# cosmicBboy/movenet

Measured on AMD Instinct MI355X. Metric: autoregressive audio samples/sec (16 kHz, 30-layer WaveNet, whole job), higher is better.
Workload: dtype f32

## Files before the change

movenet_amd/csrc/generate_fold.hip:

```cpp
#include <cstdlib>

#include "common.h"
#include "gen_common.h"
#include "pipe_common.h"

namespace mvn {

namespace fold {
constexpr int C = 64, Q = 256, NT = 512, LPS = 3;
constexpr int KQ = 4, KPER = 16, NF4 = 4;
constexpr int MAT_F = 2 * C * C;
enum { M_A0 = 0, M_A0P, M_A1, M_A2, M_B2P,
       M_B1, M_B1P, M_B2, M_RR, M_RS,
       M_WP0, M_WP1, M_WP2, M_SS,
       N_MAT };
constexpr int N_LDS_MAT = 4;
constexpr int V_CB1 = 0, V_CB2 = 2 * C, V_BSP = 4 * C, V_BR0 = 5 * C, V_BS0 = 6 * C, V_BR1 = 7 * C,
              V_BS1 = 8 * C, V_BR2 = 9 * C, VEC_F = 10 * C;
constexpr int STAGE_F = N_MAT * MAT_F + VEC_F;
constexpr int CTX_LAYER_F = MAT_F + 2 * C;
constexpr int EMB_F = 2 * Q * C;
constexpr int W1_F = Q * C, W2_F = Q * Q, WSL_F = C * C;
constexpr int HEAD_F = W1_F + Q + W2_F + Q + WSL_F + C;
constexpr int GRAN = 3 * C;
constexpr int LDS_FLOATS = N_LDS_MAT * MAT_F + 1536 + 16;
constexpr int GMAX = 8;
constexpr int PFS_F = 8;
constexpr int LDS_FLOATS_MULTI = LDS_FLOATS + GMAX * C * PFS_F;
}

struct FoldMat {
  v2f w[16];
};
__device__ __forceinline__ void fold_load(FoldMat &m, const float *sec, int t) {
#pragma unroll
  for (int i = 0; i < 8; ++i) {
    const f4 v = ((const f4 *)sec)[i * 256 + t];
    m.w[2 * i] = v2f{v.x, v.y};
    m.w[2 * i + 1] = v2f{v.z, v.w};
  }
}
__device__ __forceinline__ v2f pk_fma_hi(v2f w, v2f xpair, v2f acc) {
  asm("v_pk_fma_f32 %0, %1, %2, %0 op_sel:[0,1,0]" : "+v"(acc) : "v"(w), "v"(xpair));
  return acc;
}
__device__ __forceinline__ v2f pk_mul_hi(v2f w, v2f xpair) {
  v2f r;
  asm("v_pk_mul_f32 %0, %1, %2 op_sel:[0,1]" : "=v"(r) : "v"(w), "v"(xpair));
  return r;
}
template <bool INIT>
__device__ __forceinline__ void pair_acc(v2f (&acc)[4], const v2f (&w)[16], const f4 (&x)[4]) {
#pragma unroll
  for (int i = 0; i < 4; ++i) {
    if (INIT && i == 0) {
      acc[0] = w[0] * v2f{x[0].x, x[0].x};
      acc[1] = w[1] * v2f{x[0].y, x[0].y};
      acc[2] = w[2] * v2f{x[0].z, x[0].z};
      acc[3] = pk_mul_hi(w[3], v2f{x[0].z, x[0].w});
    } else {
      acc[0] = __builtin_elementwise_fma(w[4 * i], v2f{x[i].x, x[i].x}, acc[0]);
      acc[1] = __builtin_elementwise_fma(w[4 * i + 1], v2f{x[i].y, x[i].y}, acc[1]);
      acc[2] = __builtin_elementwise_fma(w[4 * i + 2], v2f{x[i].z, x[i].z}, acc[2]);
      acc[3] = pk_fma_hi(w[4 * i + 3], v2f{x[i].z, x[i].w}, acc[3]);
    }
  }
}
__device__ __forceinline__ v2f pair_sum(const v2f (&acc)[4]) { return (acc[0] + acc[2]) + (acc[1] + acc[3]); }
template <int H>
__device__ __forceinline__ float split_dot(const v2f (&w)[16], const f4 (&x)[4]) {
  v2f a0 = w[8 * H] * v2f{x[0].x, x[0].y}, a1 = w[8 * H + 1] * v2f{x[0].z, x[0].w};
  v2f a2 = w[8 * H + 2] * v2f{x[1].x, x[1].y}, a3 = w[8 * H + 3] * v2f{x[1].z, x[1].w};
  a0 = __builtin_elementwise_fma(w[8 * H + 4], v2f{x[2].x, x[2].y}, a0);
  a1 = __builtin_elementwise_fma(w[8 * H + 5], v2f{x[2].z, x[2].w}, a1);
  a2 = __builtin_elementwise_fma(w[8 * H + 6], v2f{x[3].x, x[3].y}, a2);
  a3 = __builtin_elementwise_fma(w[8 * H + 7], v2f{x[3].z, x[3].w}, a3);
  const v2f t = (a0 + a2) + (a1 + a3);
  return t.x + t.y;
}

typedef __attribute__((address_space(3))) float lds_f;
typedef float vf4 __attribute__((ext_vector_type(4)));
typedef __attribute__((address_space(3))) vf4 lds_f4;
__device__ __forceinline__ f4 lds_load4(unsigned addr) {
  const vf4 v = *(const lds_f4 *)(uintptr_t)addr;
  f4 r;
  r.x = v.x; r.y = v.y; r.z = v.z; r.w = v.w;
  return r;
}
__device__ __forceinline__ unsigned lds_addr(const float *p) { return (unsigned)(uintptr_t)(lds_f *)p; }
#define LDSF(addr, off) (*(lds_f *)(uintptr_t)((addr) + 4u * (unsigned)(off)))
template <int N4>
__device__ __forceinline__ void ldsv(f4 (&x)[N4], unsigned addr, int off) {
#pragma unroll
  for (int i = 0; i < N4; ++i) x[i] = lds_load4(addr + 4u * (unsigned)off + 16u * i);
}

__device__ __forceinline__ v2f pair_dot_lds(unsigned waddr, unsigned xaddr) {
  v2f acc[4];
#pragma unroll
  for (int i = 0; i < 4; ++i) {
    const f4 wa = lds_load4(waddr + 4096u * (2 * i)), wb = lds_load4(waddr + 4096u * (2 * i + 1));
    const f4 x = lds_load4(xaddr + 16u * i);
    if (i == 0) {
      acc[0] = v2f{wa.x, wa.y} * v2f{x.x, x.x};
      acc[1] = v2f{wa.z, wa.w} * v2f{x.y, x.y};
      acc[2] = v2f{wb.x, wb.y} * v2f{x.z, x.z};
      acc[3] = pk_mul_hi(v2f{wb.z, wb.w}, v2f{x.z, x.w});
    } else {
      acc[0] = __builtin_elementwise_fma(v2f{wa.x, wa.y}, v2f{x.x, x.x}, acc[0]);
      acc[1] = __builtin_elementwise_fma(v2f{wa.z, wa.w}, v2f{x.y, x.y}, acc[1]);
      acc[2] = __builtin_elementwise_fma(v2f{wb.x, wb.y}, v2f{x.z, x.z}, acc[2]);
      acc[3] = pk_fma_hi(v2f{wb.z, wb.w}, v2f{x.z, x.w}, acc[3]);
    }
  }
  return pair_sum(acc);
}
template <int H>
__device__ __forceinline__ float split_dot_lds(unsigned waddr, unsigned xaddr) {
  f4 w[4], x[4];
#pragma unroll
  for (int i = 0; i < 4; ++i) {
    w[i] = lds_load4(waddr + 4096u * (4 * H + i));
    x[i] = lds_load4(xaddr + 16u * i);
  }
  v2f a0 = v2f{w[0].x, w[0].y} * v2f{x[0].x, x[0].y}, a1 = v2f{w[0].z, w[0].w} * v2f{x[0].z, x[0].w};
  v2f a2 = v2f{w[1].x, w[1].y} * v2f{x[1].x, x[1].y}, a3 = v2f{w[1].z, w[1].w} * v2f{x[1].z, x[1].w};
  a0 = __builtin_elementwise_fma(v2f{w[2].x, w[2].y}, v2f{x[2].x, x[2].y}, a0);
  a1 = __builtin_elementwise_fma(v2f{w[2].z, w[2].w}, v2f{x[2].z, x[2].w}, a1);
  a2 = __builtin_elementwise_fma(v2f{w[3].x, w[3].y}, v2f{x[3].x, x[3].y}, a2);
  a3 = __builtin_elementwise_fma(v2f{w[3].z, w[3].w}, v2f{x[3].z, x[3].w}, a3);
  const v2f t = (a0 + a2) + (a1 + a3);
  return t.x + t.y;
}

template <bool MULTI>
__global__ __launch_bounds__(512, 2) void gen_fold_kernel(GenArgs a, u64 *hand, unsigned *err, int NS, int nb, int nseq) {
  using namespace fold;
  extern __shared__ __attribute__((aligned(16))) float smem[];
  const int tid = threadIdx.x, lane = tid & 63, wave = tid >> 6;
  const int xcd = blockIdx.x & 7, slot = blockIdx.x >> 3;
  const int in_xcd = (PIPE_XCD_CUS / NS) * NS;
  int b, s;
  if (slot < in_xcd) {
    b = xcd + 8 * (slot / NS);
    s = slot % NS;
  } else {
    const int idx = xcd * (PIPE_XCD_CUS - in_xcd) + (slot - in_xcd);
    b = 8 * (PIPE_XCD_CUS / NS) + idx / NS;
    s = idx % NS;
  }
  if (b >= nb) return;
  if (__hip_atomic_load(err, __ATOMIC_RELAXED, __HIP_MEMORY_SCOPE_AGENT) != 0) return;
  const int L = a.L;
  const int s_next = s + 1 == NS ? 0 : s + 1;
  const int G = MULTI ? (nseq - b + nb - 1) / nb : 1;
  int bq = b;
  u64 *inbox = hand + ((size_t)b * NS + s) * GRAN;
  u64 *outbox = hand + ((size_t)b * NS + s_next) * GRAN;
  int *iflag = (int *)(smem + LDS_FLOATS - 16);
  float *pfs = smem + LDS_FLOATS;
  const bool fast_edge = pipe_edge_is_fast(err + 16, b, s, s_next, NS, iflag);

  if (s < NS - 1) {
    const int l0 = s * LPS, nl = min(LPS, L - l0);
    const bool chain = tid < 256;
    const int t = tid & 255, c = t >> 2, kq = t & 3;
    const bool lead = kq == 0;
    float *lmat = smem;
    constexpr int O_XP = 0;
    constexpr int O_ZL = C;
    constexpr int O_Z0 = 2 * C, O_Z1 = 3 * C;
    constexpr int O_X0 = 4 * C;
    constexpr int O_B1 = 5 * C, O_B2 = 7 * C;
    constexpr int O_PAST = 9 * C;
    constexpr int O_CTX = 12 * C;
    constexpr int O_VEC = 13 * C;
    float *vec = smem + N_LDS_MAT * MAT_F;
    unsigned vc = lds_addr(vec) + 4u * c;
    unsigned vq = lds_addr(vec) + 4u * KPER * kq;
    asm volatile("" : "+v"(vc), "+v"(vq));
    u64 *ob = outbox + c;
    const u64 *ibs = inbox + 2 * C + c;
    float *ring = a.state + (size_t)b * a.state_per_seq;
    auto bind = [&](int g) {
      bq = b + g * nb;
      inbox = hand + ((size_t)bq * NS + s) * GRAN;
      outbox = hand + ((size_t)bq * NS + s_next) * GRAN;
      ob = outbox + c;
      ibs = inbox + 2 * C + c;
      ring = a.state + (size_t)bq * a.state_per_seq;
    };
    const float *sec = a.w + EMB_F + (size_t)s * STAGE_F;
    const float *vecs = sec + N_MAT * MAT_F;

    FoldMat m0, m1, m2, m3, m4;
    {
      const int first = chain ? M_A0 : M_B1;
      fold_load(m0, sec + (size_t)(first + 0) * MAT_F, t);
      fold_load(m1, sec + (size_t)(first + 1) * MAT_F, t);
      fold_load(m2, sec + (size_t)(first + 2) * MAT_F, t);
      fold_load(m3, sec + (size_t)(first + 3) * MAT_F, t);
      fold_load(m4, sec + (size_t)(first + 4) * MAT_F, t);
      const f4 *src = (const f4 *)(sec + (size_t)M_WP0 * MAT_F);
      for (int i = tid; i < N_LDS_MAT * MAT_F / 4; i += NT) ((f4 *)lmat)[i] = src[i];
    }
    float pf[LPS], pg[LPS];
    float (&xs)[LPS] = pf;
    int doff[LPS], dmask[LPS];
    for (int i = tid; i < VEC_F; i += NT) vec[O_VEC + i] = vecs[i];
#pragma unroll
    for (int j = 0; j < LPS; ++j) {
      pf[j] = 0.f; pg[j] = 0.f;
      const int l = l0 + j;
      dmask[j] = j < nl ? (1 << (l % a.layer_size)) - 1 : 0;
      doff[j] = j < nl ? ring_offset(l, a.layer_size, C) : 0;
    }

    float popv[LPS] = {0.f, 0.f, 0.f};
    auto prefetch_pops = [&](int tn) {
      if (MULTI && !chain && lead) {
        int cq = c;
        asm volatile("" : "+v"(cq));
#pragma unroll
        for (int j = 0; j < LPS; ++j)
          if (j < nl) popv[j] = ring_load(ring + doff[j] + cq + (tn & dmask[j]) * C);
      }
    };
    auto precompute = [&](int tn, bool push, bool popped) {
      int tq = t;
      asm volatile("" : "+v"(tq));
      const int cq = tq >> 2, kk = tq & 3;
      if (!chain && lead) {
#pragma unroll
        for (int j = 0; j < LPS; ++j)
          if (j < nl) {
            float *base = ring + doff[j] + cq;
            if (push) base[((tn - 1) & dmask[j]) * C] = xs[j];
            const float pv = (push && dmask[j] == 0) ? xs[j]
                             : (MULTI && popped) ? popv[j] : ring_load(base + (tn & dmask[j]) * C);
            vec[O_PAST + j * C + cq] = pv;
          }
      }
      if (a.ctx_tm && chain && tq < C) vec[O_CTX + tq] = a.ctx_tm[(size_t)bq * a.ctx_stride_b + (size_t)tn * C + tq];
      __syncthreads();
      if (chain) {
        const unsigned wm = lds_addr(lmat) + 16u * tq, xq = lds_addr(vec) + 4u * (O_PAST + KPER * kk);
        const v2f p0 = pair_dot_lds(wm, xq);
        const v2f p1 = pair_dot_lds(wm + 4u * MAT_F, xq + 4u * C);
        const v2f p2 = pair_dot_lds(wm + 8u * MAT_F, xq + 8u * C);
        pf[0] = chan_sum<KQ>(p0.x);
        pg[0] = chan_sum<KQ>(p0.y);
        pf[1] = chan_sum<KQ>(p1.x) + vec[O_VEC + V_CB1 + cq];
        pg[1] = chan_sum<KQ>(p1.y) + vec[O_VEC + V_CB1 + C + cq];
        pf[2] = chan_sum<KQ>(p2.x) + vec[O_VEC + V_CB2 + cq];
        pg[2] = chan_sum<KQ>(p2.y) + vec[O_VEC + V_CB2 + C + cq];
        if (a.ctx_tm) {
#pragma unroll
          for (int j = 0; j < LPS; ++j)
            if (j < nl) {
              const float *wc = a.wctx + (size_t)(l0 + j) * CTX_LAYER_F;
              pf[j] += chan_sum<KQ>(dot_stream<NF4>((const f4 *)wc, 256, tq, vec + O_CTX + KPER * kk)) + wc[MAT_F + cq];
              pg[j] += chan_sum<KQ>(dot_stream<NF4>((const f4 *)wc + NF4 * 256, 256, tq, vec + O_CTX + KPER * kk)) +
                       wc[MAT_F + C + cq];
            }
        }
      }
    };
    auto save_pf = [&](int g) {
      if (MULTI && chain && lead) {
        float *q = pfs + ((size_t)g * C + c) * PFS_F;
        *(f4 *)q = f4{pf[0], pg[0], pf[1], pg[1]};
        *(v2f *)(q + 4) = v2f{pf[2], pg[2]};
      }
    };
    auto load_pf = [&](int g) {
      if (MULTI && chain) {
        const float *q = pfs + ((size_t)g * C + c) * PFS_F;
        const f4 v = *(const f4 *)q;
        const v2f w = *(const v2f *)(q + 4);
        pf[0] = v.x; pg[0] = v.y; pf[1] = v.z; pg[1] = v.w; pf[2] = w.x; pg[2] = w.y;
      }
    };
    __syncthreads();
    if (MULTI) {
      for (int g = 0; g < G; ++g) {
        bind(g);
        precompute(a.t_begin, false, false);
        save_pf(g);
        __syncthreads();
      }
    } else {
      precompute(a.t_begin, false, false);
    }

    bool alive = true;
    for (int ts = a.t_begin; ts < a.t_end && alive; ++ts)
    for (int g = 0; g < G; ++g) {
      if (MULTI) {
        bind(g);
        if (ts + 1 < a.t_end) prefetch_pops(ts + 1);
      }
      const unsigned epoch = (unsigned)(ts - a.t_begin + 1);
      if (wave == 0) {
        float v[2];
        const bool ok = wait_inbox<2>(inbox, epoch, err, v);
        if (ok) {
          float *dst = vec + 2 * lane;
          dst[0] = v[0];
          dst[1] = v[1];
        }
        if (lane == 0) iflag[0] = ok ? 1 : 0;
      }
      lds_barrier();
      MVN_STAMP(b, s, ts - a.t_begin, 0);
      load_pf(g);
      float xv = 0.f;
      MVN_FINE(b, s, ts - a.t_begin, 0, 0);
      if (chain) {
        f4 xa[NF4], xb[NF4];
        ldsv<NF4>(xa, vq, O_XP);
        ldsv<NF4>(xb, vq, O_ZL);
        v2f acc[4];
        pair_acc<true>(acc, m0.w, xa);
        pair_acc<false>(acc, m1.w, xb);
        const v2f fg = pair_sum(acc);
        const float f = chan_sum<KQ>(fg.x) + pf[0];
        const float g = chan_sum<KQ>(fg.y) + pg[0];
        const float z = gate_fast(f, g);
        if (lead) LDSF(vc, O_Z0) = z;
        MVN_FINE(b, s, ts - a.t_begin, 1, 0);
      } else {
        f4 xa[NF4], xb[NF4];
        ldsv<NF4>(xa, vq, O_XP);
        ldsv<NF4>(xb, vq, O_ZL);
        v2f acc[4];
        pair_acc<true>(acc, m0.w, xa);
        pair_acc<false>(acc, m1.w, xb);
        const v2f fg = pair_sum(acc);
        float r = split_dot<0>(m3.w, xb);
        const float f = chan_sum<KQ>(fg.x);
        const float g = chan_sum<KQ>(fg.y);
        r = chan_sum<KQ>(r);
        if (lead) {
          xv = LDSF(vc, O_XP) + r;
          LDSF(vc, O_X0) = xv;
          xs[0] = xv;
          LDSF(vc, O_B1) = f;
          LDSF(vc, O_B1 + C) = g;
        }
        MVN_FINE(b, s, ts - a.t_begin, 6, 256);
      }
      lds_barrier();
      MVN_FINE(b, s, ts - a.t_begin, 2, 0);
      v2f b2 = {0.f, 0.f};
      if (chain) {
        f4 xz[NF4];
        ldsv<NF4>(xz, vq, O_Z0);
        v2f acc[4], acc2[4];
        pair_acc<true>(acc, m2.w, xz);
        pair_acc<true>(acc2, m4.w, xz);
        const v2f fg = pair_sum(acc);
        b2 = pair_sum(acc2);
        asm volatile("" : "+v"(b2));
        const float f = chan_sum<KQ>(fg.x) + (LDSF(vc, O_B1) + pf[1]);
        const float g = chan_sum<KQ>(fg.y) + (LDSF(vc, O_B1 + C) + pg[1]);
        const float z = gate_fast(f, g);
        if (lead) LDSF(vc, O_Z1) = z;
        MVN_FINE(b, s, ts - a.t_begin, 3, 0);
      } else {
        f4 xa[NF4], xz[NF4];
        ldsv<NF4>(xa, vq, O_X0);
        ldsv<NF4>(xz, vq, O_Z0);
        const float br0 = LDSF(vc, O_VEC + V_BR0);
        v2f acc[4];
        pair_acc<true>(acc, m2.w, xa);
        const v2f fg = pair_sum(acc);
        float r = split_dot<1>(m3.w, xz);
        const float f = chan_sum<KQ>(fg.x);
        const float g = chan_sum<KQ>(fg.y);
        r = chan_sum<KQ>(r);
        if (lead) {
          LDSF(vc, O_B2) = f;
          LDSF(vc, O_B2 + C) = g;
          xv = (xv + br0) + r;
          xs[1] = xv;
        }
        MVN_FINE(b, s, ts - a.t_begin, 7, 256);
      }
      lds_barrier();
      MVN_FINE(b, s, ts - a.t_begin, 4, 0);
      if (chain) {
        f4 xz[NF4];
        ldsv<NF4>(xz, vq, O_Z1);
        v2f acc[4];
        pair_acc<true>(acc, m3.w, xz);
        const v2f fg = pair_sum(acc) + b2;
        const float f = chan_sum<KQ>(fg.x) + (LDSF(vc, O_B2) + pf[2]);
        const float g = chan_sum<KQ>(fg.y) + (LDSF(vc, O_B2 + C) + pg[2]);
        const float z = gate_fast(f, g);
        if (lead) put_granule(ob + C, epoch, z, fast_edge);
        MVN_FINE(b, s, ts - a.t_begin, 5, 0);
      } else {
        const u64 sk_peek = peek_granule(ibs);
        f4 xz[NF4];
        ldsv<NF4>(xz, vq, O_Z1);
        const float br1 = LDSF(vc, O_VEC + V_BR1), br2 = LDSF(vc, O_VEC + V_BR2);
        float r = split_dot<0>(m4.w, xz);
        r = chan_sum<KQ>(r);
        if (lead) {
          xv = (xv + br1) + r;
          xs[2] = xv;
          put_granule(ob, epoch, xv + br2, fast_edge);
        }
        float k1 = split_dot<1>(m4.w, xz);
        unsigned wss = lds_addr(lmat + 3 * MAT_F) + 16u * t;
        asm volatile("" : "+v"(wss));
        float kp = split_dot_lds<0>(wss, vq + 4u * O_ZL);
        float k0 = split_dot_lds<1>(wss, vq + 4u * O_Z0);
        kp = chan_sum<KQ>(kp);
        k0 = chan_sum<KQ>(k0);
        k1 = chan_sum<KQ>(k1);
        if (lead) {
          const float bsp = LDSF(vc, O_VEC + V_BSP), bs0 = LDSF(vc, O_VEC + V_BS0), bs1 = LDSF(vc, O_VEC + V_BS1);
          const float skin = (unsigned)(sk_peek >> 32) == epoch ? __uint_as_float((unsigned)sk_peek)
                                                                : wait_granule(ibs, epoch, err);
          put_granule(ob + 2 * C, epoch, ((skin + (kp + bsp)) + (k0 + bs0)) + (k1 + bs1), fast_edge);
        }
      }
      MVN_STAMP(b, s, ts - a.t_begin, 1);
      lds_barrier();
      if (iflag[0] == 0) {
        alive = false;
        break;
      }
      if (ts + 1 < a.t_end) {
        precompute(ts + 1, true, true);
        save_pf(g);
      } else if (!chain && lead) {
        int cq = c;
        asm volatile("" : "+v"(cq));
#pragma unroll
        for (int j = 0; j < LPS; ++j)
          if (j < nl) ring[doff[j] + cq + (ts & dmask[j]) * C] = xs[j];
      }
    }
    return;
  }

  {
    float *tab = smem;
    float *vec = smem + N_LDS_MAT * MAT_F;
    float *zlb = vec;
    float *a0 = zlb + C;
    float *a1 = a0 + C;
    float *lgb = a1 + Q;
    const float *E0 = tab, *E1 = tab + Q * C;
    const float *hw = a.w + EMB_F + (size_t)(NS - 1) * STAGE_F;
    const f4 *W1p = (const f4 *)hw, *W2p = (const f4 *)(hw + W1_F + Q);
    const float *b1 = hw + W1_F, *b2 = hw + W1_F + Q + W2_F;
    const f4 *WSp = (const f4 *)(hw + W1_F + Q + W2_F + Q);
    const float *bsl = hw + W1_F + Q + W2_F + Q + WSL_F;
    int *hidx = (int *)pfs;

    const int o1 = tid >> 1, q1 = tid & 1, og = tid >> 3, q2 = tid & 7;
    v2f wsl[4], w1[16], w2[4][16];
    {
      const f4 *src = (const f4 *)a.w;
      f4 *dst = (f4 *)tab;
      for (int i = tid; i < EMB_F / 4; i += NT) dst[i] = src[i];
      loadn<2>(wsl, WSp, NT, tid);
      loadn<8>(w1, W1p, NT, tid);
#pragma unroll
      for (int r = 0; r < 4; ++r) loadn<8>(w2[r], W2p + r * 8 * NT, NT, tid);
    }
    const float b1r = b1[o1];
    const float b2r = b2[4 * og + (q2 & 3)];
    const float bslr = bsl[og];
    __syncthreads();

    auto await = [&](const u64 *inbox, unsigned epoch) {
      float v[2];
      const bool ok = wait_inbox64(inbox + C, epoch, err, v);
      if (ok && lane < 32) {
        zlb[2 * lane] = v[0];
        zlb[2 * lane + 1] = v[1];
      }
      return ok;
    };
    auto logits = [&](const u64 *inbox, unsigned epoch, bool do_head) {
      const u64 sk_peek = peek_granule(inbox + 2 * C + og);
      float sv = 0.f;
      if (do_head) {
        f4 x[2];
        ldsn<2>(x, zlb + 8 * q2);
        sv = dotn<2>(wsl, x);
        sv = quad_sum(sv);
        sv += other_quad(sv);
      }
      float skin = 0.f;
      if (q2 == 0)
        skin = (unsigned)(sk_peek >> 32) == epoch ? __uint_as_float((unsigned)sk_peek)
                                                  : wait_granule(inbox + 2 * C + og, epoch, err);
      if (!do_head) return;
      if (q2 == 0) a0[og] = leaky(skin + (sv + bslr));
      lds_barrier();
      {
        f4 x[8];
        ldsn<8>(x, a0 + 32 * q1);
        float hsum = dotn<8>(w1, x);
        hsum += dpp_mov<DPP_XOR1>(hsum);
        if (q1 == 0) a1[o1] = leaky(hsum + b1r);
      }
      lds_barrier();
      head_conv2_f32(w2, a1, lgb, og, q2, b2r);
      lds_barrier();
    };
    head_loop<C, GRAN, MULTI, 2>(a, hand, NS, nb, b, G, fast_edge, E0, E1, iflag, hidx, lgb, await, logits);
  }
}

struct FoldLayers {
  const float *fw[4], *gw[4], *rw[4], *rb[4], *sw[4], *sb[4];
};
__device__ __forceinline__ double fold_wc(const FoldLayers &p, int j, int row, int k) {
  return p.fw[j] ? (double)fg_elem(p.fw[j], p.gw[j], fold::C, row, fold::C + k) : 0.0;
}
__device__ __forceinline__ double fold_wr(const FoldLayers &p, int j, int o, int k) {
  return p.rw[j] ? (double)p.rw[j][(size_t)o * fold::C + k] : 0.0;
}
__device__ __forceinline__ double fold_br(const FoldLayers &p, int j, int o) { return p.rb[j] ? (double)p.rb[j][o] : 0.0; }

__global__ void pack_fold_stage_kernel(FoldLayers p, float *__restrict__ dst) {
  using namespace fold;
  const int i = blockIdx.x * blockDim.x + threadIdx.x;
  if (i >= STAGE_F) return;
  if (i >= N_MAT * MAT_F) {
    const int o = i - N_MAT * MAT_F;
    double v = 0.0;
    if (o < V_CB2) {
      for (int m = 0; m < C; ++m) v += fold_wc(p, 2, o - V_CB1, m) * fold_br(p, 1, m);
    } else if (o < V_BSP) {
      for (int m = 0; m < C; ++m) v += fold_wc(p, 3, o - V_CB2, m) * (fold_br(p, 1, m) + fold_br(p, 2, m));
    } else if (o < V_BR0) v = p.sb[0] ? p.sb[0][o - V_BSP] : 0.0;
    else if (o < V_BS0) v = fold_br(p, 1, o - V_BR0);
    else if (o < V_BR1) v = p.sb[1] ? p.sb[1][o - V_BS0] : 0.0;
    else if (o < V_BS1) v = fold_br(p, 2, o - V_BR1);
    else if (o < V_BR2) v = p.sb[2] ? p.sb[2][o - V_BS1] : 0.0;
    else v = fold_br(p, 3, o - V_BR2);
    dst[i] = (float)v;
    return;
  }
  const int mat = i / MAT_F, r = i - mat * MAT_F;
  const int e = r & 3, v4 = r >> 2, t = v4 & 255, i4 = v4 >> 8;
  const bool split = mat == M_RR || mat == M_RS || mat == M_SS;
  const int row = split ? (i4 / NF4) * C + t / KQ : (e & 1) * C + t / KQ;
  const int k = KPER * (t % KQ) + (split ? 4 * (i4 % NF4) + e : 2 * i4 + (e >> 1));
  double v = 0.0;
  auto prod = [&](int jc, int jr) {
    double acc = 0.0;
    for (int m = 0; m < C; ++m) acc += fold_wc(p, jc, row, m) * fold_wr(p, jr, m, k);
    return acc;
  };
  auto ws = [&](int j, int o) { return p.sw[j] ? (double)p.sw[j][(size_t)o * C + k] : 0.0; };
  auto wp = [&](int j) { return p.fw[j] ? (double)fg_elem(p.fw[j], p.gw[j], C, row, k) : 0.0; };
  switch (mat) {
    case M_A0: v = fold_wc(p, 1, row, k); break;
    case M_A0P: v = prod(1, 0); break;
    case M_A1: v = prod(2, 1); break;
    case M_A2: v = prod(3, 2); break;
    case M_B2P: v = prod(3, 1); break;
    case M_B1: v = fold_wc(p, 2, row, k); break;
    case M_B1P: v = prod(2, 0); break;
    case M_B2: v = fold_wc(p, 3, row, k); break;
    case M_RR: v = row < C ? fold_wr(p, 0, row, k) : fold_wr(p, 1, row - C, k); break;
    case M_RS: v = row < C ? fold_wr(p, 2, row, k) : ws(2, row - C); break;
    case M_WP0: v = wp(1); break;
    case M_WP1: v = wp(2); break;
    case M_WP2: v = wp(3); break;
    case M_SS: v = row < C ? ws(0, row) : ws(1, row - C); break;
  }
  dst[i] = (float)v;
}

__global__ void pack_fold_head_kernel(const float *w1, const float *b1, const float *w2, const float *b2,
                                      const float *sw_last, const float *sb_last, float *__restrict__ dst, int qm) {
  using namespace fold;
  const int i = blockIdx.x * blockDim.x + threadIdx.x;
  if (pack_head_f32(i, C, C / 2, qm, w1, b1, w2, b2, dst)) return;
  if (i < W1_F + Q + W2_F + Q + WSL_F) {
    const int ii = i - (W1_F + Q + W2_F + Q);
    const int e = ii & 3, v = ii >> 2, tid = v & (NT - 1), i2 = v >> 9;
    dst[i] = sw_last ? sw_last[(size_t)(tid >> 3) * C + 8 * (tid & 7) + 4 * i2 + e] : 0.f;
  } else if (i < HEAD_F) {
    dst[i] = sb_last ? sb_last[i - (W1_F + Q + W2_F + Q + WSL_F)] : 0.f;
  }
}

bool fold_ok(const mvn_dims *d) {
  return d->residual_channels == 64 && d->skip_channels == 64 && head_q_ok(d->input_channels) &&
         n_layers(d) >= 1 && (n_layers(d) + fold::LPS - 1) / fold::LPS + 1 <= PIPE_XCD_CUS;
// ... 75 lines not shown
```

movenet_amd/csrc/pipe_common.h:

```cpp
#pragma once
#include <cstdio>
#include <cstdlib>
#include <cstring>

#include "common.h"
#include "gen_common.h"

namespace mvn {

typedef unsigned long long u64;
typedef float4 f4;

constexpr int PIPE_XCD_CUS = 32;
constexpr unsigned PIPE_SPIN_LIMIT = 1u << 23;
constexpr int HEAD_Q = 256, HEAD_NT = 512;

inline bool pipe_profiler_attached() {
  for (const char *v : {"ROCP_TOOL_LIBRARIES", "ROCPROFILER_REGISTER_FORCE_LOAD", "HSA_TOOLS_LIB", "ROCP_METRICS"})
    if (const char *e = getenv(v))
      if (e[0]) return true;
  if (const char *pre = getenv("LD_PRELOAD"))
    if (strstr(pre, "rocprof")) return true;
  bool found = false;
  if (FILE *f = fopen("/proc/self/maps", "r")) {
    char line[512];
    while (!found && fgets(line, sizeof line, f))
      found = strstr(line, "librocprofiler-sdk-tool") || strstr(line, "librocprofiler64");
    fclose(f);
  }
  return found;
}
inline bool pipe_cooperative_launch() {
  static const bool on = [] {
    const char *e = getenv("MOVENET_PIPE_COOPERATIVE_LAUNCH");
    if (e && (e[0] == '0' || e[0] == '1')) return e[0] == '1';
    return !pipe_profiler_attached();
  }();
  return on;
}

__host__ __device__ inline int pipe_span(int NS) { return (NS + PIPE_XCD_CUS - 1) / PIPE_XCD_CUS; }
inline int pipe_pipelines_of(int NS) {
  return NS <= PIPE_XCD_CUS ? 8 * (PIPE_XCD_CUS / NS) : 8 / pipe_span(NS);
}
inline int pipe_grid_slots(int NS, int pipes) {
  return NS <= PIPE_XCD_CUS ? (pipes + 7) / 8 * NS : (NS + pipe_span(NS) - 1) / pipe_span(NS);
}
__device__ __forceinline__ bool pipe_place(unsigned block, int NS, int &b, int &s) {
  const int xcd = block & 7, slot = block >> 3;
  if (NS <= PIPE_XCD_CUS) {
    b = xcd + 8 * (slot / NS);
    s = slot % NS;
    return true;
  }
  const int XS = pipe_span(NS), SPX = (NS + XS - 1) / XS;
  b = xcd / XS;
  s = (xcd % XS) * SPX + slot;
  return slot < SPX && s < NS;
}

__device__ __forceinline__ bool pipe_edge_is_fast(unsigned *xcc, int b, int s, int s_next, int NS, int *iflag) {
  const unsigned mine = (__builtin_amdgcn_s_getreg((3 << 11) | 20) & 0xF) + 1;
  if (threadIdx.x == 0) {
    __hip_atomic_store(xcc + b * NS + s, mine, __ATOMIC_RELAXED, __HIP_MEMORY_SCOPE_AGENT);
    unsigned other = 0;
    for (unsigned spins = 0; spins < (1u << 20) && other == 0; ++spins) {
      other = __hip_atomic_load(xcc + b * NS + s_next, __ATOMIC_RELAXED, __HIP_MEMORY_SCOPE_AGENT);
      if (other == 0) __builtin_amdgcn_s_sleep(8);
    }
    iflag[3] = (other == mine) ? 1 : 0;
  }
  __syncthreads();
  const bool fast = iflag[3] != 0;
  __syncthreads();
  return fast;
}

#ifdef MVN_PIPE_STAMPS
static __device__ unsigned long long g_stamps[16][16][64][4];
#define MVN_STAMP(bb, ss, step, which)                                              \
  do {                                                                              \
    if ((bb) < 16 && (ss) < 16 && (step) < 64 && threadIdx.x == 0) {                \
      g_stamps[bb][ss][step][which] = __builtin_amdgcn_s_memrealtime();             \
      g_stamps[bb][ss][step][2 + (which)] = __builtin_amdgcn_s_memtime();           \
    }                                                                               \
  } while (0)
static __device__ unsigned long long g_fine[16][16][64][8];
#define MVN_FINE(bb, ss, step, slot, who)                                           \
  do {                                                                              \
    if ((bb) < 16 && (ss) < 16 && (step) < 64 && threadIdx.x == (who))              \
      g_fine[bb][ss][step][slot] = __builtin_amdgcn_s_memtime();                    \
  } while (0)
template <class T>
inline int debug_read(const T &sym, unsigned long long *out, size_t n, const char *what) {
  if (n > sizeof(T) / 8) n = sizeof(T) / 8;
  return check_hip(hipMemcpyFromSymbol(out, HIP_SYMBOL(sym), n * 8), what);
}
#else
#define MVN_STAMP(bb, ss, step, which) do {} while (0)
#define MVN_FINE(bb, ss, step, slot, who) do {} while (0)
#endif

__device__ __forceinline__ void put_granule(u64 *g, unsigned epoch, float v, bool same_xcd) {
  const u64 x = ((u64)epoch << 32) | (u64)__float_as_uint(v);
  if (same_xcd)
    __hip_atomic_store(g, x, __ATOMIC_RELAXED, __HIP_MEMORY_SCOPE_WORKGROUP);
  else
    __hip_atomic_store(g, x, __ATOMIC_RELAXED, __HIP_MEMORY_SCOPE_AGENT);
}

typedef unsigned v4u __attribute__((ext_vector_type(4)));

__device__ __forceinline__ int poll16(const u64 *p, unsigned epoch, float &v0, float &v1) {
  int st;
  unsigned r0, r1;
  u64 tmp;
  asm volatile(
      "s_movk_i32 %[st], 64\n\t"
      "global_load_dwordx4 v[240:243], %[p], off sc1\n"
      "1:\n\t"
      "global_load_dwordx4 v[244:247], %[p], off sc1\n\t"
      "s_waitcnt vmcnt(1)\n\t"
      "v_cmp_eq_u32 vcc, %[ep], v241\n\t"
      "v_cmp_eq_u32 %[t], %[ep], v243\n\t"
      "s_and_b64 vcc, vcc, %[t]\n\t"
      "s_cmp_eq_u64 vcc, exec\n\t"
      "s_cbranch_scc1 2f\n\t"
      "global_load_dwordx4 v[240:243], %[p], off sc1\n\t"
      "s_waitcnt vmcnt(1)\n\t"
      "v_cmp_eq_u32 vcc, %[ep], v245\n\t"
      "v_cmp_eq_u32 %[t], %[ep], v247\n\t"
      "s_and_b64 vcc, vcc, %[t]\n\t"
      "s_cmp_eq_u64 vcc, exec\n\t"
      "s_cbranch_scc1 3f\n\t"
      "s_sub_u32 %[st], %[st], 1\n\t"
      "s_cmp_lg_u32 %[st], 0\n\t"
      "s_cbranch_scc1 1b\n\t"
      "s_waitcnt vmcnt(0)\n\t"
      "s_mov_b32 %[st], 0\n\t"
      "s_branch 4f\n"
      "2:\n\t"
      "s_waitcnt vmcnt(0)\n\t"
      "v_mov_b32 %[r0], v240\n\t"
      "v_mov_b32 %[r1], v242\n\t"
      "s_mov_b32 %[st], 1\n\t"
      "s_branch 4f\n"
      "3:\n\t"
      "s_waitcnt vmcnt(0)\n\t"
      "v_mov_b32 %[r0], v244\n\t"
      "v_mov_b32 %[r1], v246\n\t"
      "s_mov_b32 %[st], 1\n"
      "4:\n"
      : [st] "=&s"(st), [r0] "=&v"(r0), [r1] "=&v"(r1), [t] "=&s"(tmp)
      : [p] "v"(p), [ep] "s"(epoch)
      : "vcc", "scc", "memory", "v240", "v241", "v242", "v243", "v244", "v245", "v246", "v247");
  v0 = __uint_as_float(r0);
  v1 = __uint_as_float(r1);
  return st;
}
__device__ __forceinline__ bool wait16(const u64 *p, unsigned epoch, unsigned *err, float &v0, float &v1) {
  for (unsigned calls = 1;; ++calls) {
    if (poll16(p, epoch, v0, v1)) return true;
    const unsigned e = __hip_atomic_load(err, __ATOMIC_RELAXED, __HIP_MEMORY_SCOPE_AGENT);
    if (e != 0 || calls > PIPE_SPIN_LIMIT / 128) {
      if ((threadIdx.x & 63) == 0) __hip_atomic_store(err, 1u, __ATOMIC_RELAXED, __HIP_MEMORY_SCOPE_AGENT);
      return false;
    }
  }
}

// ... 276 lines not shown
  const float m = wave_max_dpp(fmaxf(fmaxf(lg[0], lg[1]), fmaxf(lg[2], lg[3])));
  float e[4];
#pragma unroll
  for (int k = 0; k < 4; ++k) e[k] = __expf(lg[k] - m);
  const float sm = wave_sum_dpp((e[0] + e[1]) + (e[2] + e[3]));
  const float rs = __builtin_amdgcn_rcpf(sm) * (temperature > 0.f ? __builtin_amdgcn_rcpf(temperature) : 1.0f);
  float p[4];
#pragma unroll
  for (int k = 0; k < 4; ++k) p[k] = e[k] * rs;
  const float m2 = rs;
#pragma unroll
  for (int k = 0; k < 4; ++k) e[k] = 4 * lane + k < Q ? __expf(p[k] - m2) : 0.f;
  const float s2sum = wave_sum_dpp((e[0] + e[1]) + (e[2] + e[3]));
  const float rs2 = __builtin_amdgcn_rcpf(s2sum);
#pragma unroll
  for (int k = 0; k < 4; ++k) p[k] = e[k] * rs2;

  int pick;
  if (temperature > 0.f) {
    const float lsum = (p[0] + p[1]) + (p[2] + p[3]);
    float incl = lsum;
    incl += dpp_mov<0x111>(incl);
    incl += dpp_mov<0x112>(incl);
    incl += dpp_mov<0x114>(incl);
    incl += dpp_mov<0x118>(incl);
    {
      const float r0 = lane_value(incl, 15), r1 = lane_value(incl, 31), r2 = lane_value(incl, 47);
      const int row = lane >> 4;
      incl += row == 0 ? 0.f : row == 1 ? r0 : row == 2 ? r0 + r1 : (r0 + r1) + r2;
    }
    const float total = lane_value(incl, 63);
    const float target = uniform * total;
    const float cdf = incl - lsum;
    int cand = Q - 1;
    bool hit = false;
#pragma unroll
    for (int k = 3; k >= 0; --k) {
      const float c_k = cdf + (k == 0 ? p[0] : k == 1 ? p[0] + p[1]
                                              : k == 2 ? (p[0] + p[1]) + p[2]
                                                       : ((p[0] + p[1]) + p[2]) + p[3]);
      if (c_k > target) {
        cand = 4 * lane + k;
        hit = true;
      }
    }
    const unsigned long long lanes = __builtin_amdgcn_ballot_w64(hit);
    pick = lanes ? __builtin_amdgcn_readlane(cand, __builtin_ctzll(lanes)) : Q - 1;
  } else {
    float bv = p[0];
    int bi = 4 * lane;
#pragma unroll
    for (int k = 1; k < 4; ++k)
      if (p[k] > bv) {
        bv = p[k];
        bi = 4 * lane + k;
      }
    argmax_take(bv, bi, dpp_mov<DPP_XOR1>(bv), dpp_movi<DPP_XOR1>(bi));
    argmax_take(bv, bi, dpp_mov<DPP_XOR2>(bv), dpp_movi<DPP_XOR2>(bi));
    argmax_take(bv, bi, dpp_mov<DPP_HALF_MIRROR>(bv), dpp_movi<DPP_HALF_MIRROR>(bi));
    argmax_take(bv, bi, dpp_mov<DPP_MIRROR>(bv), dpp_movi<DPP_MIRROR>(bi));
    float rv = lane_value(bv, 0);
    pick = __builtin_amdgcn_readlane(bi, 0);
#pragma unroll
    for (int row = 16; row < 64; row += 16)
      argmax_take(rv, pick, lane_value(bv, row), __builtin_amdgcn_readlane(bi, row));
  }
  return pick;
}

__device__ __forceinline__ void head_conv2_f32(const v2f (&w2)[4][16], const float *a1, float *lgb, int og, int q2,
                                               float b2r) {
  f4 x[8];
  ldsn<8>(x, a1 + 32 * q2);
  float s0 = dotn<8>(w2[0], x), s1 = dotn<8>(w2[1], x);
  float s2 = dotn<8>(w2[2], x), s3 = dotn<8>(w2[3], x);
  s0 = quad_sum(s0); s0 += other_quad(s0);
  s1 = quad_sum(s1); s1 += other_quad(s1);
  s2 = quad_sum(s2); s2 += other_quad(s2);
  s3 = quad_sum(s3); s3 += other_quad(s3);
  const int sel = q2 & 3;
  if (q2 < 4) lgb[4 * og + sel] = (sel == 0 ? s0 : sel == 1 ? s1 : sel == 2 ? s2 : s3) + b2r;
}

template <int C, int GRAN, bool MULTI, int NZ, class Await, class Logits>
__device__ __forceinline__ void head_loop(const GenArgs &a, u64 *hand, int NS, int nb, int b, int G, bool fast_edge,
                                          const float *E0, const float *E1, int *iflag, int *hidx, const float *lgb,
                                          Await await, Logits logits) {
  static_assert(GRAN == (1 + NZ) * C, "residual stream + NZ zero lanes");
  const int lane = threadIdx.x & 63, wave = threadIdx.x >> 6, s = NS - 1;
  int bq;
  const u64 *inbox;
  u64 *outbox;
  int32_t *samples;
  auto bind = [&](int g) {
    bq = b + g * nb;
    inbox = hand + ((size_t)bq * NS + s) * GRAN;
    outbox = hand + (size_t)bq * NS * GRAN;
    samples = a.samples + (size_t)bq * a.stride;
  };
  int idx_cur = 0, idx_prev = -1;
  auto send_h0 = [&](unsigned ep) {
    const int ic = min(max(idx_cur, 0), a.Q - 1), ip = min(idx_prev, a.Q - 1);
#pragma unroll
    for (int j = 0; j < C / 64; ++j) {
      const int ch = lane + 64 * j;
      float v = E1[ic * C + ch];
      if (ip >= 0) v += E0[ip * C + ch];
      put_granule(outbox + ch, ep, v, fast_edge);
#pragma unroll
      for (int z = 1; z <= NZ; ++z) put_granule(outbox + z * C + ch, ep, 0.f, fast_edge);
    }
  };
  for (int g = 0; g < G; ++g) {
    bind(g);
    if (wave == 0) {
      idx_cur = samples[a.t_begin];
      idx_prev = a.t_begin > 0 ? samples[a.t_begin - 1] : -1;
      if (a.t_begin < a.t_end) send_h0(1u);
      MVN_STAMP(b, s, 0, 1);
      if (MULTI && lane == 0) {
        hidx[2 * g] = idx_cur;
        hidx[2 * g + 1] = idx_prev;
      }
    }
  }
  if (MULTI) __syncthreads();

  for (int ts = a.t_begin; ts < a.t_end; ++ts)
  for (int g = 0; g < G; ++g) {
    if (MULTI) {
      bind(g);
      if (wave == 0) {
        idx_cur = hidx[2 * g];
        idx_prev = hidx[2 * g + 1];
      }
    }
    const unsigned epoch = (unsigned)(ts - a.t_begin + 1);
    const int u = ts + 1;
    const bool want_out = (a.logits_out || a.choices_out) && u >= a.logits_t0;
    const bool do_head = u < a.n_total && (u >= a.n_given || want_out);
    int next_idx = 0;
    float uni = 0.f;
    if (wave == 0 && a.temperature > 0.f) {
      uni = philox_uniform(a.seed, (uint32_t)u, (uint32_t)bq);
      asm volatile("" : "+v"(uni));
    }
    if (wave == 0) {
      if (u < a.n_given) next_idx = samples[u];
      const bool ok = await(inbox, epoch);
      if (lane == 0) iflag[0] = ok ? 1 : 0;
    }
    lds_barrier();
    MVN_STAMP(b, s, ts - a.t_begin, 0);
    logits(inbox, epoch, do_head);
    if (wave == 0) {
      int pick = 0;
      if (do_head) {
        const f4 lv = ((const f4 *)lgb)[lane];
        const float lg[4] = {lv.x, lv.y, lv.z, lv.w};
        if (a.logits_out && u >= a.logits_t0 && 4 * lane < a.Q)
          ((f4 *)(a.logits_out + ((size_t)bq * (a.n_total - a.logits_t0) + (u - a.logits_t0)) * a.Q))[lane] = lv;
        pick = choose_class(lg, a.temperature, uni, lane, a.Q);
        if (u >= a.n_given) next_idx = pick;
      }
      idx_prev = idx_cur;
      idx_cur = next_idx;
      if (ts + 1 < a.t_end) send_h0(epoch + 1);
      MVN_STAMP(b, s, ts + 1 - a.t_begin, 1);
      if (do_head && lane == 0) {
        if (a.choices_out && u >= a.logits_t0) a.choices_out[(size_t)bq * a.n_total + u] = pick;
        if (u >= a.n_given) samples[u] = pick;
      }
      if (MULTI && lane == 0) {
        hidx[2 * g] = idx_cur;
        hidx[2 * g + 1] = idx_prev;
      }
    }
    if (iflag[0] == 0) return;
  }
}

__device__ __forceinline__ bool pack_head_f32(int i, int C, int W1N, int qm, const float *w1, const float *b1,
                                              const float *w2, const float *b2, float *__restrict__ dst) {
  constexpr int Q = HEAD_Q, NT = HEAD_NT;
  const int W1_F = Q * C, W2_F = Q * Q;
  if (i < W1_F) {
    const int e = i & 3, v = i >> 2, tid = v & (NT - 1), i4 = v >> 9;
    const int o = tid >> 1;
    dst[i] = o < qm ? w1[(size_t)o * C + W1N * (tid & 1) + 4 * i4 + e] : 0.f;
  } else if (i < W1_F + Q) {
    dst[i] = i - W1_F < qm ? b1[i - W1_F] : 0.f;
  } else if (i < W1_F + Q + W2_F) {
    const int ii = i - W1_F - Q;
    const int e = ii & 3, v = ii >> 2, tid = v & (NT - 1), rest = v >> 9, r = rest >> 3, i8 = rest & 7;
    const int o = 4 * (tid >> 3) + r, k = 32 * (tid & 7) + 4 * i8 + e;
    dst[i] = (o < qm && k < qm) ? w2[(size_t)o * qm + k] : 0.f;
  } else if (i < W1_F + Q + W2_F + Q) {
    const int o = i - W1_F - Q - W2_F;
    dst[i] = o < qm ? b2[o] : -INFINITY;
  } else {
    return false;
  }
  return true;
}

}
```

Baseline: 1.077 million.

## Specialize first pipeline stage to skip zero lanes and reorder last-stage residual send

Turns the layer stage body into a lambda templated on whether the stage is the first one. The first stage now skips the zero-valued ZL and skip-input lanes: no m1 load, no ZL matvec, no skip-input wait, and a 64-lane inbox wait. The head stops sending those zero granules (NZ_SENT=0). The residual update for layer 1 moves into the final phase. The second-to-last stage computes the skip sum before the residual, and it no longer sends the residual because the head does not use it. This shortens the critical path and cuts handoff traffic, at the cost of more code paths and more fine-grained timing probes.

```diff
diff --git a/movenet_amd/csrc/generate_fold.hip b/movenet_amd/csrc/generate_fold.hip
--- a/movenet_amd/csrc/generate_fold.hip
+++ b/movenet_amd/csrc/generate_fold.hip
@@ -1,4 +1,5 @@
 #include <cstdlib>
+#include <type_traits>
 
 #include "common.h"
 #include "gen_common.h"
@@ -162,7 +163,9 @@
   float *pfs = smem + LDS_FLOATS;
   const bool fast_edge = pipe_edge_is_fast(err + 16, b, s, s_next, NS, iflag);
 
-  if (s < NS - 1) {
+  auto layer_stage = [&](auto first_stage) {
+    constexpr bool FIRST = decltype(first_stage)::value;
+    const bool last = s == NS - 2;
     const int l0 = s * LPS, nl = min(LPS, L - l0);
     const bool chain = tid < 256;
     const int t = tid & 255, c = t >> 2, kq = t & 3;
@@ -194,11 +197,11 @@
     const float *sec = a.w + EMB_F + (size_t)s * STAGE_F;
     const float *vecs = sec + N_MAT * MAT_F;
 
-    FoldMat m0, m1, m2, m3, m4;
+    FoldMat m0, m1 = {}, m2, m3, m4;
     {
       const int first = chain ? M_A0 : M_B1;
       fold_load(m0, sec + (size_t)(first + 0) * MAT_F, t);
-      fold_load(m1, sec + (size_t)(first + 1) * MAT_F, t);
+      if (!FIRST) fold_load(m1, sec + (size_t)(first + 1) * MAT_F, t);
       fold_load(m2, sec + (size_t)(first + 2) * MAT_F, t);
       fold_load(m3, sec + (size_t)(first + 3) * MAT_F, t);
       fold_load(m4, sec + (size_t)(first + 4) * MAT_F, t);
@@ -304,8 +307,8 @@
       const unsigned epoch = (unsigned)(ts - a.t_begin + 1);
       if (wave == 0) {
         float v[2];
-        const bool ok = wait_inbox<2>(inbox, epoch, err, v);
-        if (ok) {
+        const bool ok = FIRST ? wait_inbox64(inbox, epoch, err, v) : wait_inbox<2>(inbox, epoch, err, v);
+        if (ok && (!FIRST || lane < 32)) {
           float *dst = vec + 2 * lane;
           dst[0] = v[0];
           dst[1] = v[1];
@@ -320,10 +323,10 @@
       if (chain) {
         f4 xa[NF4], xb[NF4];
         ldsv<NF4>(xa, vq, O_XP);
-        ldsv<NF4>(xb, vq, O_ZL);
+        if (!FIRST) ldsv<NF4>(xb, vq, O_ZL);
         v2f acc[4];
         pair_acc<true>(acc, m0.w, xa);
-        pair_acc<false>(acc, m1.w, xb);
+        if (!FIRST) pair_acc<false>(acc, m1.w, xb);
         const v2f fg = pair_sum(acc);
         const float f = chan_sum<KQ>(fg.x) + pf[0];
         const float g = chan_sum<KQ>(fg.y) + pg[0];
@@ -333,15 +336,16 @@
       } else {
         f4 xa[NF4], xb[NF4];
         ldsv<NF4>(xa, vq, O_XP);
-        ldsv<NF4>(xb, vq, O_ZL);
+        if (!FIRST) ldsv<NF4>(xb, vq, O_ZL);
         v2f acc[4];
         pair_acc<true>(acc, m0.w, xa);
-        pair_acc<false>(acc, m1.w, xb);
+        if (!FIRST) pair_acc<false>(acc, m1.w, xb);
         const v2f fg = pair_sum(acc);
-        float r = split_dot<0>(m3.w, xb);
+        float r = 0.f;
+        if (!FIRST) r = split_dot<0>(m3.w, xb);
         const float f = chan_sum<KQ>(fg.x);
         const float g = chan_sum<KQ>(fg.y);
-        r = chan_sum<KQ>(r);
+        if (!FIRST) r = chan_sum<KQ>(r);
         if (lead) {
           xv = LDSF(vc, O_XP) + r;
           LDSF(vc, O_X0) = xv;
@@ -369,22 +373,16 @@
         if (lead) LDSF(vc, O_Z1) = z;
         MVN_FINE(b, s, ts - a.t_begin, 3, 0);
       } else {
-        f4 xa[NF4], xz[NF4];
+        f4 xa[NF4];
         ldsv<NF4>(xa, vq, O_X0);
-        ldsv<NF4>(xz, vq, O_Z0);
-        const float br0 = LDSF(vc, O_VEC + V_BR0);
         v2f acc[4];
         pair_acc<true>(acc, m2.w, xa);
         const v2f fg = pair_sum(acc);
-        float r = split_dot<1>(m3.w, xz);
         const float f = chan_sum<KQ>(fg.x);
         const float g = chan_sum<KQ>(fg.y);
-        r = chan_sum<KQ>(r);
         if (lead) {
           LDSF(vc, O_B2) = f;
           LDSF(vc, O_B2 + C) = g;
-          xv = (xv + br0) + r;
-          xs[1] = xv;
         }
         MVN_FINE(b, s, ts - a.t_begin, 7, 256);
       }
@@ -402,30 +400,56 @@
         if (lead) put_granule(ob + C, epoch, z, fast_edge);
         MVN_FINE(b, s, ts - a.t_begin, 5, 0);
       } else {
-        const u64 sk_peek = peek_granule(ibs);
+        u64 sk_peek = 0;
+        if (!FIRST) sk_peek = peek_granule(ibs);
         f4 xz[NF4];
         ldsv<NF4>(xz, vq, O_Z1);
-        const float br1 = LDSF(vc, O_VEC + V_BR1), br2 = LDSF(vc, O_VEC + V_BR2);
-        float r = split_dot<0>(m4.w, xz);
-        r = chan_sum<KQ>(r);
-        if (lead) {
-          xv = (xv + br1) + r;
-          xs[2] = xv;
-          put_granule(ob, epoch, xv + br2, fast_edge);
-        }
-        float k1 = split_dot<1>(m4.w, xz);
-        unsigned wss = lds_addr(lmat + 3 * MAT_F) + 16u * t;
-        asm volatile("" : "+v"(wss));
-        float kp = split_dot_lds<0>(wss, vq + 4u * O_ZL);
-        float k0 = split_dot_lds<1>(wss, vq + 4u * O_Z0);
-        kp = chan_sum<KQ>(kp);
-        k0 = chan_sum<KQ>(k0);
-        k1 = chan_sum<KQ>(k1);
-        if (lead) {
-          const float bsp = LDSF(vc, O_VEC + V_BSP), bs0 = LDSF(vc, O_VEC + V_BS0), bs1 = LDSF(vc, O_VEC + V_BS1);
-          const float skin = (unsigned)(sk_peek >> 32) == epoch ? __uint_as_float((unsigned)sk_peek)
-                                                                : wait_granule(ibs, epoch, err);
-          put_granule(ob + 2 * C, epoch, ((skin + (kp + bsp)) + (k0 + bs0)) + (k1 + bs1), fast_edge);
+        auto stream = [&](bool send) {
+          f4 xz0[NF4];
+          ldsv<NF4>(xz0, vq, O_Z0);
+          const float br0 = LDSF(vc, O_VEC + V_BR0), br1 = LDSF(vc, O_VEC + V_BR1), br2 = LDSF(vc, O_VEC + V_BR2);
+          float r0 = split_dot<1>(m3.w, xz0);
+          float r = split_dot<0>(m4.w, xz);
+          r0 = chan_sum<KQ>(r0);
+          r = chan_sum<KQ>(r);
+          if (lead) {
+            xv = (xv + br0) + r0;
+            xs[1] = xv;
+            xv = (xv + br1) + r;
+            xs[2] = xv;
+            if (send) put_granule(ob, epoch, xv + br2, fast_edge);
+          }
+          MVN_FINE(b, s, ts - a.t_begin, 8, 256);
+        };
+        auto skip = [&] {
+          float k1 = split_dot<1>(m4.w, xz);
+          unsigned wss = lds_addr(lmat + 3 * MAT_F) + 16u * t;
+          asm volatile("" : "+v"(wss));
+          float kp = 0.f;
+          if (!FIRST) kp = split_dot_lds<0>(wss, vq + 4u * O_ZL);
+          float k0 = split_dot_lds<1>(wss, vq + 4u * O_Z0);
+          if (!FIRST) kp = chan_sum<KQ>(kp);
+          k0 = chan_sum<KQ>(k0);
+          k1 = chan_sum<KQ>(k1);
+          if (lead) {
+            const float bs0 = LDSF(vc, O_VEC + V_BS0), bs1 = LDSF(vc, O_VEC + V_BS1);
+            float sk0 = 0.f;
+            if (!FIRST) {
+              const float bsp = LDSF(vc, O_VEC + V_BSP);
+              const float skin = (unsigned)(sk_peek >> 32) == epoch ? __uint_as_float((unsigned)sk_peek)
+                                                                    : wait_granule(ibs, epoch, err);
+              sk0 = skin + (kp + bsp);
+            }
+            put_granule(ob + 2 * C, epoch, (sk0 + (k0 + bs0)) + (k1 + bs1), fast_edge);
+          }
+          MVN_FINE(b, s, ts - a.t_begin, 9, 256);
+        };
+        if (last) {
+          skip();
+          stream(false);
+        } else {
+          stream(true);
+          skip();
         }
       }
       MVN_STAMP(b, s, ts - a.t_begin, 1);
@@ -445,6 +469,12 @@
           if (j < nl) ring[doff[j] + cq + (ts & dmask[j]) * C] = xs[j];
       }
     }
+  };
+  if (s < NS - 1) {
+    if (s == 0)
+      layer_stage(std::true_type{});
+    else
+      layer_stage(std::false_type{});
     return;
   }
 
@@ -489,6 +519,7 @@
       return ok;
     };
     auto logits = [&](const u64 *inbox, unsigned epoch, bool do_head) {
+      MVN_FINE(b, NS - 1, epoch - 1, 0, 0);
       const u64 sk_peek = peek_granule(inbox + 2 * C + og);
       float sv = 0.f;
       if (do_head) {
@@ -502,6 +533,7 @@
       if (q2 == 0)
         skin = (unsigned)(sk_peek >> 32) == epoch ? __uint_as_float((unsigned)sk_peek)
                                                   : wait_granule(inbox + 2 * C + og, epoch, err);
+      MVN_FINE(b, NS - 1, epoch - 1, 1, 0);
       if (!do_head) return;
       if (q2 == 0) a0[og] = leaky(skin + (sv + bslr));
       lds_barrier();
@@ -513,10 +545,12 @@
         if (q1 == 0) a1[o1] = leaky(hsum + b1r);
       }
       lds_barrier();
+      MVN_FINE(b, NS - 1, epoch - 1, 3, 0);
       head_conv2_f32(w2, a1, lgb, og, q2, b2r);
       lds_barrier();
+      MVN_FINE(b, NS - 1, epoch - 1, 4, 0);
     };
-    head_loop<C, GRAN, MULTI, 2>(a, hand, NS, nb, b, G, fast_edge, E0, E1, iflag, hidx, lgb, await, logits);
+    head_loop<C, GRAN, MULTI, 2, 0>(a, hand, NS, nb, b, G, fast_edge, E0, E1, iflag, hidx, lgb, await, logits);
   }
 }
 
diff --git a/movenet_amd/csrc/pipe_common.h b/movenet_amd/csrc/pipe_common.h
--- a/movenet_amd/csrc/pipe_common.h
+++ b/movenet_amd/csrc/pipe_common.h
@@ -85,7 +85,7 @@
       g_stamps[bb][ss][step][2 + (which)] = __builtin_amdgcn_s_memtime();           \
     }                                                                               \
   } while (0)
-static __device__ unsigned long long g_fine[16][16][64][8];
+static __device__ unsigned long long g_fine[16][16][64][12];
 #define MVN_FINE(bb, ss, step, slot, who)                                           \
   do {                                                                              \
     if ((bb) < 16 && (ss) < 16 && (step) < 64 && threadIdx.x == (who))              \
@@ -528,11 +528,11 @@
   if (q2 < 4) lgb[4 * og + sel] = (sel == 0 ? s0 : sel == 1 ? s1 : sel == 2 ? s2 : s3) + b2r;
 }
 
-template <int C, int GRAN, bool MULTI, int NZ, class Await, class Logits>
+template <int C, int GRAN, bool MULTI, int NZ, int NZ_SENT = NZ, class Await, class Logits>
 __device__ __forceinline__ void head_loop(const GenArgs &a, u64 *hand, int NS, int nb, int b, int G, bool fast_edge,
                                           const float *E0, const float *E1, int *iflag, int *hidx, const float *lgb,
                                           Await await, Logits logits) {
-  static_assert(GRAN == (1 + NZ) * C, "residual stream + NZ zero lanes");
+  static_assert(GRAN == (1 + NZ) * C && NZ_SENT <= NZ, "residual stream + NZ zero lanes");
   const int lane = threadIdx.x & 63, wave = threadIdx.x >> 6, s = NS - 1;
   int bq;
   const u64 *inbox;
@@ -554,7 +554,7 @@
       if (ip >= 0) v += E0[ip * C + ch];
       put_granule(outbox + ch, ep, v, fast_edge);
 #pragma unroll
-      for (int z = 1; z <= NZ; ++z) put_granule(outbox + z * C + ch, ep, 0.f, fast_edge);
+      for (int z = 1; z <= NZ_SENT; ++z) put_granule(outbox + z * C + ch, ep, 0.f, fast_edge);
     }
   };
   for (int g = 0; g < G; ++g) {
@@ -613,6 +613,7 @@
       idx_cur = next_idx;
       if (ts + 1 < a.t_end) send_h0(epoch + 1);
       MVN_STAMP(b, s, ts + 1 - a.t_begin, 1);
+      MVN_FINE(b, s, ts - a.t_begin, 5, 0);
       if (do_head && lane == 0) {
         if (a.choices_out && u >= a.logits_t0) a.choices_out[(size_t)bq * a.n_total + u] = pick;
         if (u >= a.n_given) samples[u] = pick;
```

New measurement: 1.116 million (median of 6 runs). +3.6%, better.
